# google-research/multinerf

Measured on NVIDIA H100. Metric: train-step rays/sec @16384 rays x (64+64+32) samples, higher is better.
Workload: dtype bf16

## Files before the change

### multinerf_b200/csrc/chain.cu

```cuda
#include <stdlib.h>
#include <string.h>

#include <algorithm>

#include "tc_common.cuh"

namespace mnrf {

constexpr int CH_W = 256;
constexpr int CH_ROWS = 128;
constexpr int CH_KBLK = CH_ROWS * 128;
constexpr int CH_WBLK = CH_W * 128;
constexpr int CH_SLOT = CH_WBLK + CH_KBLK;
constexpr int CH_SLOTS = 3;
constexpr int CH_ACT = 4 * CH_KBLK;
constexpr int CH_THREADS = 384;
constexpr int CH_MAX_LAYERS = MNRF_CHAIN_MAX_LAYERS;
constexpr int CH_SMEM = CH_ACT + CH_SLOTS * CH_SLOT + CH_MAX_LAYERS * CH_W * 4  + 256  +
                        1024 ;
static_assert(CH_SMEM <= 232448, "shared memory budget");

struct alignas(64) ChainMaps {
  CUtensorMap stream;
  CUtensorMap w[CH_MAX_LAYERS];
  CUtensorMap out[CH_MAX_LAYERS];
};

struct ChainLayer {
  int n_stream, stream_col0, stream_kb0;
  int n_res, res_kb0;
  int store;
  const float* bias;
  uint32_t* maskbits;
  int64_t ldmaskbits;
  float* colsum;
};

struct ChainParams {
  int num_layers;
  int64_t m;
  int64_t num_units;
  ChainLayer layer[CH_MAX_LAYERS];
  const float* head_w;
  const float* head_b;
  float* head_out;
};

__device__ __forceinline__ uint32_t pack_bf16_relu(float lo, float hi) {
  uint32_t r;
  asm("cvt.rn.relu.bf16x2.f32 %0, %1, %2;" : "=r"(r) : "f"(hi), "f"(lo));
  return r;
}

template <int MODE, int NH>
__global__ void __launch_bounds__(CH_THREADS, 1)
mlp_chain_kernel(const __grid_constant__ ChainMaps maps, const ChainParams p) {
  extern __shared__ uint8_t smem_dyn[];
  uint8_t* smem = reinterpret_cast<uint8_t*>((reinterpret_cast<uintptr_t>(smem_dyn) + 1023) & ~uintptr_t(1023));
  uint8_t* act = smem;
  uint8_t* ring = smem + CH_ACT;
  float* cs_s = reinterpret_cast<float*>(ring + CH_SLOTS * CH_SLOT);
  uint64_t* full_bar = reinterpret_cast<uint64_t*>(cs_s + CH_MAX_LAYERS * CH_W);
  uint64_t* empty_bar = full_bar + CH_SLOTS;

  const int warp = threadIdx.x >> 5;
  const int lane = threadIdx.x & 31;
  const int wg = threadIdx.x >> 7;

  if (threadIdx.x == 0) {
    bool any_stream = false;
    for (int j = 0; j < p.num_layers; ++j) {
      prefetch_tmap(&maps.w[j]);
      if (p.layer[j].store) prefetch_tmap(&maps.out[j]);
      any_stream |= p.layer[j].n_stream > 0;
    }
    if (any_stream) prefetch_tmap(&maps.stream);
    for (int i = 0; i < CH_SLOTS; ++i) { mbar_init(&full_bar[i], 1); mbar_init(&empty_bar[i], 8); }
    fence_barrier_init();
  }
  if (MODE == 1)
    for (int i = threadIdx.x; i < CH_MAX_LAYERS * CH_W; i += CH_THREADS) cs_s[i] = 0.f;
  __syncthreads();
  pdl_launch_dependents();
  pdl_wait();

  if (wg == 0) {
    setmaxnreg_dec<40>();
    if (threadIdx.x == 0) {
      uint32_t slot = 0, phase = 0;
      for (int64_t unit = blockIdx.x; unit < p.num_units; unit += gridDim.x) {
        const int row0 = (int)(unit * CH_ROWS);
        for (int j = 0; j < p.num_layers; ++j) {
          const ChainLayer& L = p.layer[j];
          for (int s = 0; s < L.n_res + L.n_stream; ++s) {
            const bool streamed = s >= L.n_res;
            const int si = s - L.n_res;
            mbar_wait(&empty_bar[slot], phase ^ 1, 1);
            mbar_expect_tx(&full_bar[slot], streamed ? CH_SLOT : CH_WBLK);
            uint8_t* sl = ring + slot * CH_SLOT;
            const int kb = streamed ? L.stream_kb0 + si : L.res_kb0 + s;
            tma_load_2d(sl, &maps.w[j], &full_bar[slot], kb * 64, 0);
            if (streamed) tma_load_2d(sl + CH_WBLK, &maps.stream, &full_bar[slot], L.stream_col0 + si * 64, row0);
            if (++slot == CH_SLOTS) { slot = 0; phase ^= 1; }
          }
        }
      }
    }
  } else {
    setmaxnreg_inc<232>();
    const int c = wg - 1;
    const int w = warp & 3;
    const int r_in = 64 * c + 16 * w + (lane >> 2);
    const int cq = 2 * (lane & 3);
    const uint32_t ring_s = smem_u32(ring), act_s = smem_u32(act);
    const bool lead = (threadIdx.x & 127) == 0;
    uint32_t slot = 0, phase = 0;
    float acc[CH_W / 2];
    for (int64_t unit = blockIdx.x; unit < p.num_units; unit += gridDim.x) {
      for (int j = 0; j < p.num_layers; ++j) {
        const ChainLayer& L = p.layer[j];
        const bool last = (j == p.num_layers - 1);
        const bool do_head = (MODE == 0) && last && p.head_w != nullptr;
        int prev = -1;
        fence_acc(acc);
        for (int s = 0; s < L.n_res + L.n_stream; ++s) {
          const bool streamed = s >= L.n_res;
          mbar_wait(&full_bar[slot], phase, 3);
          const uint32_t sl = ring_s + slot * CH_SLOT;
          const uint32_t a0 = (streamed ? sl + CH_WBLK : act_s + s * CH_KBLK) + c * (64 * 128);
          wgmma_fence();
#pragma unroll
          for (int k = 0; k < 64 / WGMMA_K; ++k)
            Wgmma<CH_W, 0, 0>::mma(acc, make_smem_desc(a0 + k * (WGMMA_K * 2), 0, 1024),
                                   make_smem_desc(sl + k * (WGMMA_K * 2), 0, 1024), (s > 0 || k > 0) ? 1u : 0u);
          wgmma_commit();
          wgmma_wait<1>();
          if (prev >= 0 && lane == 0) mbar_arrive(&empty_bar[prev]);
          prev = (int)slot;
          if (++slot == CH_SLOTS) { slot = 0; phase ^= 1; }
        }
        wgmma_wait<0>();
        fence_acc(acc);
        if (prev >= 0 && lane == 0) mbar_arrive(&empty_bar[prev]);

        if (lead) tma_store_wait_read<0>();
        named_bar_sync(1 + c, 128);
        int64_t rows[2];
        bool row_ok[2];
#pragma unroll
        for (int h = 0; h < 2; ++h) {
          rows[h] = unit * CH_ROWS + r_in + 8 * h;
          row_ok[h] = rows[h] < p.m;
        }
        uint32_t bits[2] = {0u, 0u};
        float hdot[NH][2];
#pragma unroll
        for (int o = 0; o < NH; ++o) hdot[o][0] = hdot[o][1] = 0.f;
#pragma unroll
        for (int i = 0; i < CH_W / 8; ++i) {
          const int col = 8 * i + cq;
          float v[2][2];
#pragma unroll
          for (int h = 0; h < 2; ++h) { v[h][0] = acc[4 * i + 2 * h]; v[h][1] = acc[4 * i + 2 * h + 1]; }
          uint32_t o[2];
          if (MODE == 0) {
            const float2 b = __ldg(reinterpret_cast<const float2*>(L.bias + col));
#pragma unroll
            for (int h = 0; h < 2; ++h) {
              v[h][0] += b.x;
              v[h][1] += b.y;
              bits[h] |= ((v[h][0] > 0.f ? 1u : 0u) | (v[h][1] > 0.f ? 2u : 0u)) << (col & 31);
              o[h] = pack_bf16_relu(v[h][0], v[h][1]);
            }
            if (do_head) {
#pragma unroll
              for (int oo = 0; oo < NH; ++oo) {
                const float2 hw = __ldg(reinterpret_cast<const float2*>(p.head_w + oo * CH_W + col));
#pragma unroll
                for (int h = 0; h < 2; ++h) hdot[oo][h] += bf16_lo(o[h]) * hw.x + bf16_hi(o[h]) * hw.y;
              }
            }
          } else {
#pragma unroll
            for (int h = 0; h < 2; ++h) {
              if (L.maskbits) {
                const uint32_t wd = row_ok[h] ? __ldg(L.maskbits + rows[h] * L.ldmaskbits + (col >> 5)) : 0u;
                if (!((wd >> (col & 31)) & 1u)) v[h][0] = 0.f;
                if (!((wd >> ((col + 1) & 31)) & 1u)) v[h][1] = 0.f;
              }
              o[h] = pack_bf16(v[h][0], v[h][1]);
            }
            if (L.colsum) {
              float s0 = v[0][0] + v[1][0], s1 = v[0][1] + v[1][1];
#pragma unroll
              for (int sh = 4; sh < 32; sh <<= 1) {
                s0 += __shfl_xor_sync(0xffffffffu, s0, sh);
                s1 += __shfl_xor_sync(0xffffffffu, s1, sh);
              }
              if (lane < 4) { atomicAdd(cs_s + j * CH_W + col, s0); atomicAdd(cs_s + j * CH_W + col + 1, s1); }
            }
          }
#pragma unroll
          for (int h = 0; h < 2; ++h) {
            const int r = r_in + 8 * h;
            st_shared_u32(act_s + (col >> 6) * CH_KBLK + r * 128 + ((((col & 63) >> 3) ^ (r & 7)) << 4) + (cq << 1), o[h]);
// ... 131 lines not shown
```

### multinerf_b200/csrc/gemm_tc.cu

```cuda
#include <cuda.h>

#include <stdlib.h>
#include <string.h>

#include <algorithm>

#include "tc_common.cuh"

namespace mnrf {

constexpr int BLOCK_M = 128;
constexpr int BLOCK_K = 64;
constexpr int A_STAGE_BYTES = BLOCK_M * BLOCK_K * 2;
constexpr int NUM_THREADS = 384;
constexpr int CS_MAX = 1024;
constexpr int gemm_stages(int bn) { return bn == 256 ? 4 : bn == 128 ? 6 : 8; }
constexpr int STAGING_BLOCK_BYTES = 64 * 128;
constexpr int staging_blocks(int mode, int bn, bool ts) {
  return !ts ? 0 : (mode == MNRF_GEMM_FWD && bn >= 128) ? 2 : 1;
}
constexpr int mask_words(int bn) { return bn >= 128 ? bn / 32 : 0; }
constexpr int MASK_BUFS = 2;
constexpr int dgrad_smem_bytes(int bn) { return 8 * bn * 4 + MASK_BUFS * BLOCK_M * mask_words(bn) * 4; }
constexpr int SIDE_SCRATCH = 96 * 8;
constexpr int smem_bytes(int mode, int bn, bool ts, bool side) {
  return gemm_stages(bn) * (A_STAGE_BYTES + bn * BLOCK_K * 2) + 2 * staging_blocks(mode, bn, ts) * STAGING_BLOCK_BYTES +
         (mode == MNRF_GEMM_DGRAD ? dgrad_smem_bytes(bn) : 0) + (side ? SIDE_SCRATCH * 4 : 0) + 256  +
         1024 ;
}

struct GemmParams {
  int mode, act;
  int64_t m;
  int n, k;
  int num_m_blocks, num_n_blocks, num_splits, kblocks_per_split, num_k_blocks;
  int64_t ldc, ldmask;
  const float* bias;
  const float* rowv;
  const float* colv;
  const __nv_bfloat16* mask;
  uint32_t* maskbits;
  int64_t ldmaskbits;
  int64_t mask_mod;
  int mask_tma;
  const __nv_bfloat16* addend;
  int64_t ldadd;
  float* colsum;
  float* bsum;
  const float* side_w;
  float* side_aw;
  void* out;
};

template <int STAGES, int STAGE_BYTES, int CHUNKS, int NT, bool WEIGHTED>
__device__ __forceinline__ void wgrad_side_sums(const GemmParams& p, int t, uint32_t ring, uint64_t* full_bar,
                                                uint64_t* empty_bar, uint32_t scratch) {
  constexpr int G = NT / CHUNKS;
  constexpr int COLS = CHUNKS * 8;
  static_assert(NT % CHUNKS == 0 && NT % 32 == 0, "side-sum warps tile the chunks");
  const int lane = t & 31;
  const int c = t % CHUNKS, g0 = t / CHUNKS;
  ring += (c >> 3) * (BLOCK_K * 128) + ((c & 7) << 4);
  const int total_tiles = p.num_m_blocks * p.num_n_blocks * p.num_splits;
  const int every = WEIGHTED ? p.num_n_blocks : p.num_m_blocks;
  const int step = every * G;
  uint32_t slot = 0;
  for (int tile = blockIdx.x; tile < total_tiles; tile += gridDim.x) {
    const int n_blk = tile % p.num_n_blocks;
    const int rest = tile / p.num_n_blocks;
    const int m_blk = rest % p.num_m_blocks;
    const int split = rest / p.num_m_blocks;
    const int kb0 = split * p.kblocks_per_split;
    const int kb1 = min(p.num_k_blocks, kb0 + p.kblocks_per_split);
    const int own = WEIGHTED ? n_blk : m_blk;
    float acc[8];
#pragma unroll
    for (int e = 0; e < 8; ++e) acc[e] = 0.f;
    for (int kb = kb0; kb < kb1; ++kb, ++slot) {
      float wlo = 0.f, whi = 0.f;
      if (WEIGHTED) {
        const int r0 = kb * BLOCK_K + lane;
        if (r0 < p.k) wlo = __ldg(p.side_w + r0);
        if (r0 + 32 < p.k) whi = __ldg(p.side_w + r0 + 32);
      }
      mbar_wait(&full_bar[slot % STAGES], (slot / STAGES) & 1, 6);
      const uint32_t base = ring + (slot % STAGES) * STAGE_BYTES;
#pragma unroll(WEIGHTED ? 2 : 1)
      for (int r0 = own; r0 < BLOCK_K; r0 += step) {
        const int r = r0 + every * g0;
        float w = 1.f;
        if (WEIGHTED) {
          const float wl = __shfl_sync(0xffffffffu, wlo, r & 31), wh = __shfl_sync(0xffffffffu, whi, r & 31);
          w = r < 32 ? wl : wh;
        }
        if (r < BLOCK_K) {
          const uint4 v = ld_shared_v4((base + r * 128) ^ ((r & 7) << 4));
          const uint32_t u[4] = {v.x, v.y, v.z, v.w};
#pragma unroll
          for (int q = 0; q < 4; ++q) {
            acc[2 * q] = fmaf(w, bf16_lo(u[q]), acc[2 * q]);
            acc[2 * q + 1] = fmaf(w, bf16_hi(u[q]), acc[2 * q + 1]);
          }
        }
      }
      __syncwarp();
      if (lane == 0) mbar_arrive(&empty_bar[slot % STAGES]);
    }
    if (own < BLOCK_K && kb0 < kb1) {
      if (NT > 32) named_bar_sync(4, NT); else __syncwarp();
#pragma unroll
      for (int e = 0; e < 8; ++e) st_shared_u32(scratch + (t * 8 + e) * 4, __float_as_uint(acc[e]));
      if (NT > 32) named_bar_sync(4, NT); else __syncwarp();
      const int64_t col0 = WEIGHTED ? (int64_t)m_blk * BLOCK_M : (int64_t)n_blk * COLS;
      float* out = WEIGHTED ? p.side_aw : p.bsum;
      for (int col = t; col < COLS; col += NT) {
        if (WEIGHTED && col0 + col >= p.m) break;
        float sum = 0.f;
#pragma unroll
        for (int g = 0; g < G; ++g) sum += __uint_as_float(ld_shared_u32(scratch + (g * COLS + col) * 4));
        atomicAdd(out + col0 + col, sum);
      }
    }
  }
}

template <int MODE, int BN, bool TS, bool SIDE, bool SMOOTH = false>
__global__ void __launch_bounds__(NUM_THREADS, 1)
gemm_tc_kernel(const __grid_constant__ CUtensorMap tmap_a, const __grid_constant__ CUtensorMap tmap_b,
               const __grid_constant__ CUtensorMap tmap_c, const __grid_constant__ CUtensorMap tmap_m,
               const GemmParams p) {
  constexpr int STAGES = gemm_stages(BN);
  constexpr int B_STAGE = BN * BLOCK_K * 2;
  constexpr bool kWgrad = (MODE == MNRF_GEMM_WGRAD);
  constexpr bool kDgrad = (MODE == MNRF_GEMM_DGRAD);
  constexpr int NACC = BN / 2;
  constexpr int SB = staging_blocks(MODE, BN, TS);
  constexpr int MW = mask_words(BN);
  static_assert(SB < 2 || (BN / 64) % 2 == 0, "block j of every tile must use staging block j % SB");
  static_assert(!SIDE || kWgrad, "side sums are a WGRAD feature");
  static_assert(!SMOOTH || (TS && !kWgrad), "smooth activations are FWD / DGRAD epilogues of the staged store");
  extern __shared__ uint8_t smem_dyn[];
  uint8_t* smem = reinterpret_cast<uint8_t*>((reinterpret_cast<uintptr_t>(smem_dyn) + 1023) & ~uintptr_t(1023));
  uint8_t* smem_a = smem;
  uint8_t* smem_b = smem + STAGES * A_STAGE_BYTES;
  uint8_t* smem_c = smem_b + STAGES * B_STAGE;
  float* cs_s = reinterpret_cast<float*>(smem_c + 2 * SB * STAGING_BLOCK_BYTES);
  float* side_s = cs_s;
  uint32_t* mask_s = reinterpret_cast<uint32_t*>(cs_s + (kDgrad ? 8 * BN : SIDE ? SIDE_SCRATCH : 0));
  uint64_t* full_bar = reinterpret_cast<uint64_t*>(mask_s + (kDgrad ? MASK_BUFS * BLOCK_M * MW : 0));
  uint64_t* empty_bar = full_bar + STAGES;
  uint64_t* mask_full = empty_bar + STAGES;
  uint64_t* mask_empty = mask_full + MASK_BUFS;

  const int warp = threadIdx.x >> 5;
  const int lane = threadIdx.x & 31;
  const int wg = threadIdx.x >> 7;
  const int total_tiles = p.num_m_blocks * p.num_n_blocks * p.num_splits;
  const bool do_cs = kDgrad && p.colsum != nullptr;
  const bool mask_tma = kDgrad && p.mask_tma;

  if (threadIdx.x == 0) {
    prefetch_tmap(&tmap_a);
    prefetch_tmap(&tmap_b);
    if (TS) prefetch_tmap(&tmap_c);
    if (mask_tma) prefetch_tmap(&tmap_m);
    for (int i = 0; i < STAGES; ++i) {
      mbar_init(&full_bar[i], 1);
      mbar_init(&empty_bar[i], 8 + (!SIDE ? 0 : !p.side_aw ? 3 : p.bsum ? 3 : 2));
    }
    for (int i = 0; i < MASK_BUFS; ++i) {
      mbar_init(&mask_full[i], 1);
      mbar_init(&mask_empty[i], 8);
    }
    fence_barrier_init();
  }
  if (do_cs)
    for (int i = threadIdx.x; i < 8 * BN; i += NUM_THREADS) cs_s[i] = 0.f;
  __syncthreads();
  pdl_launch_dependents();
  pdl_wait();

  if (wg == 0) {
    setmaxnreg_dec<40>();
    if (threadIdx.x == 0) {
      const uint32_t stage_bytes = A_STAGE_BYTES + B_STAGE;
      uint32_t stage = 0, phase = 0;
      for (int tile = blockIdx.x, it = 0; tile < total_tiles; tile += gridDim.x, ++it) {
        const int n_blk = tile % p.num_n_blocks;
        const int rest = tile / p.num_n_blocks;
        const int m_blk = rest % p.num_m_blocks;
        const int split = rest / p.num_m_blocks;
        const int kb0 = split * p.kblocks_per_split;
        const int kb1 = min(p.num_k_blocks, kb0 + p.kblocks_per_split);
        if (mask_tma) {
          const int mb = it % MASK_BUFS;
          mbar_wait(&mask_empty[mb], ((it / MASK_BUFS) & 1) ^ 1, 4);
          mbar_expect_tx(&mask_full[mb], BLOCK_M * MW * 4);
          const int64_t r0 = (int64_t)m_blk * BLOCK_M;
          tma_load_2d(mask_s + mb * (BLOCK_M * MW), &tmap_m, &mask_full[mb], n_blk * (BN / 32),
                      (int)(p.mask_mod > 0 ? r0 % p.mask_mod : r0));
        }
        for (int kb = kb0; kb < kb1; ++kb) {
          mbar_wait(&empty_bar[stage], phase ^ 1, 1);
          mbar_expect_tx(&full_bar[stage], stage_bytes);
          uint8_t* sa = smem_a + stage * A_STAGE_BYTES;
          uint8_t* sb = smem_b + stage * B_STAGE;
          if (!kWgrad) {
            tma_load_2d(sa, &tmap_a, &full_bar[stage], kb * BLOCK_K, m_blk * BLOCK_M);
            tma_load_2d(sb, &tmap_b, &full_bar[stage], kb * BLOCK_K, n_blk * BN);
          } else {
#pragma unroll
            for (int a = 0; a < BLOCK_M / 64; ++a)
              tma_load_2d(sa + a * (BLOCK_K * 128), &tmap_a, &full_bar[stage], m_blk * BLOCK_M + a * 64, kb * BLOCK_K);
#pragma unroll
            for (int a = 0; a < BN / 64; ++a)
              tma_load_2d(sb + a * (BLOCK_K * 128), &tmap_b, &full_bar[stage], n_blk * BN + a * 64, kb * BLOCK_K);
          }
          if (++stage == STAGES) { stage = 0; phase ^= 1; }
        }
      }
    } else if (SIDE && warp > 0) {
      const uint32_t scratch = smem_u32(side_s);
      if (!p.side_aw) {
        wgrad_side_sums<STAGES, B_STAGE, BN / 8, 96, false>(p, threadIdx.x - 32, smem_u32(smem_b), full_bar, empty_bar,
                                                            scratch);
      } else if (warp >= 2) {
        wgrad_side_sums<STAGES, A_STAGE_BYTES, BLOCK_M / 8, 64, true>(p, threadIdx.x - 64, smem_u32(smem_a), full_bar,
                                                                      empty_bar, scratch + 32 * 8 * 4);
      } else if (p.bsum) {
        wgrad_side_sums<STAGES, B_STAGE, BN / 8, 32, false>(p, lane, smem_u32(smem_b), full_bar, empty_bar, scratch);
      }
    }
  } else {
    setmaxnreg_inc<232>();
    const int c = wg - 1;
    const int w = warp & 3;
    const int r_in = 64 * c + 16 * w + (lane >> 2);
    const int cq = 2 * (lane & 3);
    uint32_t stage = 0, phase = 0;
    float acc[NACC];
    const uint32_t cs_lane = smem_u32(cs_s) + ((warp - 4) * BN + cq + ((lane >> 2) & 1)) * 4;
    for (int tile = blockIdx.x, it = 0; tile < total_tiles; tile += gridDim.x, ++it) {
      const int n_blk = tile % p.num_n_blocks;
      const int rest = tile / p.num_n_blocks;
      const int m_blk = rest % p.num_m_blocks;
      const int split = rest / p.num_m_blocks;
      const int kb0 = split * p.kblocks_per_split;
      const int kb1 = min(p.num_k_blocks, kb0 + p.kblocks_per_split);
      int prev = -1;
      fence_acc(acc);
      for (int kb = kb0; kb < kb1; ++kb) {
        mbar_wait(&full_bar[stage], phase, 3);
        const uint32_t sa = smem_u32(smem_a + stage * A_STAGE_BYTES);
        const uint32_t sb = smem_u32(smem_b + stage * B_STAGE);
        wgmma_fence();
#pragma unroll
        for (int k = 0; k < BLOCK_K / WGMMA_K; ++k) {
          uint64_t adesc, bdesc;
          if (!kWgrad) {
            adesc = make_smem_desc(sa + c * (64 * 128) + k * (WGMMA_K * 2), 0, 1024);
            bdesc = make_smem_desc(sb + k * (WGMMA_K * 2), 0, 1024);
          } else {
            adesc = make_smem_desc(sa + c * (BLOCK_K * 128) + k * (WGMMA_K * 128), BLOCK_K * 128, 1024);
            bdesc = make_smem_desc(sb + k * (WGMMA_K * 128), BLOCK_K * 128, 1024);
          }
          Wgmma<BN, kWgrad ? 1 : 0, kWgrad ? 1 : 0>::mma(acc, adesc, bdesc, (kb > kb0 || k > 0) ? 1u : 0u);
        }
        wgmma_commit();
        wgmma_wait<1>();
        if (prev >= 0 && lane == 0) mbar_arrive(&empty_bar[prev]);
        prev = (int)stage;
        if (++stage == STAGES) { stage = 0; phase ^= 1; }
      }
      wgmma_wait<0>();
      fence_acc(acc);
      if (prev >= 0 && lane == 0) mbar_arrive(&empty_bar[prev]);

      const int ncol0 = n_blk * BN;
      if (MODE == MNRF_GEMM_WGRAD) {
#pragma unroll
        for (int h = 0; h < 2; ++h) {
          const int64_t row = (int64_t)m_blk * BLOCK_M + r_in + 8 * h;
          if (row >= p.m) continue;
          float* dst = reinterpret_cast<float*>(p.out) + row * p.ldc + ncol0 + cq;
#pragma unroll
          for (int i = 0; i < BN / 8; ++i) atomicAdd(reinterpret_cast<float2*>(dst + 8 * i), make_float2(acc[4 * i + 2 * h], acc[4 * i + 2 * h + 1]));
        }
        continue;
      }
      const bool leader = (threadIdx.x & 127) == 0;
      const uint32_t c_row = smem_u32(smem_c) + c * (SB * STAGING_BLOCK_BYTES) + (r_in - 64 * c) * 128 + (cq << 1);
      int64_t rows[2];
      bool row_ok[2];
      float rv[2] = {0.f, 0.f};
      const uint32_t* mrow[2] = {nullptr, nullptr};
#pragma unroll
      for (int h = 0; h < 2; ++h) {
        rows[h] = (int64_t)m_blk * BLOCK_M + r_in + 8 * h;
        row_ok[h] = rows[h] < p.m;
        if (MODE == MNRF_GEMM_DGRAD && row_ok[h]) {
          if (p.rowv) rv[h] = p.rowv[rows[h]];
          if (p.maskbits && !mask_tma)
            mrow[h] = p.maskbits + (p.mask_mod > 0 ? rows[h] % p.mask_mod : rows[h]) * p.ldmaskbits;
        }
      }
      const uint32_t m_row = smem_u32(mask_s) + ((it % MASK_BUFS) * BLOCK_M + r_in) * (MW * 4);
      if (mask_tma) mbar_wait(&mask_full[it % MASK_BUFS], (it / MASK_BUFS) & 1, 5);
      uint32_t bits[2] = {0u, 0u};
      uint32_t mw[2] = {0u, 0u};
#pragma unroll
      for (int i = 0; i < BN / 8; ++i) {
        const int col = ncol0 + 8 * i + cq;
        if (TS && SB == 1 && (i & 7) == 0) {
          if (leader) tma_store_wait_read<0>();
          named_bar_sync(2 + c, 128);
        }
        if (MODE == MNRF_GEMM_DGRAD && p.maskbits && (i & 3) == 0) {
#pragma unroll
          for (int h = 0; h < 2; ++h)
            mw[h] = mask_tma ? ld_shared_u32(m_row + (8 * h * MW + (i >> 2)) * 4)
                             : row_ok[h] ? __ldg(mrow[h] + (col >> 5)) : 0u;
        }
        float v[2][2];
#pragma unroll
        for (int h = 0; h < 2; ++h) { v[h][0] = acc[4 * i + 2 * h]; v[h][1] = acc[4 * i + 2 * h + 1]; }
        if (MODE == MNRF_GEMM_FWD) {
          if (p.bias) {
            const float2 b = __ldg(reinterpret_cast<const float2*>(p.bias + col));
#pragma unroll
            for (int h = 0; h < 2; ++h) { v[h][0] += b.x; v[h][1] += b.y; }
          }
          if constexpr (SMOOTH) {
#pragma unroll
            for (int h = 0; h < 2; ++h) {
              if (p.mask && row_ok[h])
                *reinterpret_cast<uint32_t*>(const_cast<__nv_bfloat16*>(p.mask) + rows[h] * p.ldmask + col) =
                    pack_bf16(v[h][0], v[h][1]);
              v[h][0] = act_fwd(p.act, v[h][0]);
              v[h][1] = act_fwd(p.act, v[h][1]);
            }
          } else if (p.act == MNRF_ACT_RELU) {
#pragma unroll
            for (int h = 0; h < 2; ++h)
#pragma unroll
              for (int e = 0; e < 2; ++e) {
                v[h][e] = fmaxf(v[h][e], 0.f);
                bits[h] |= (v[h][e] > 0.f ? 1u : 0u) << ((8 * i + cq + e) & 31);
              }
          }
        } else {
          float2 cv = make_float2(0.f, 0.f);
          if (p.rowv) cv = __ldg(reinterpret_cast<const float2*>(p.colv + col));
#pragma unroll
          for (int h = 0; h < 2; ++h) {
            if (p.rowv) { v[h][0] += rv[h] * cv.x; v[h][1] += rv[h] * cv.y; }
            if constexpr (SMOOTH) {
              if (row_ok[h]) {
                const int64_t zr = p.mask_mod > 0 ? rows[h] % p.mask_mod : rows[h];
                const uint32_t zz = __ldg(reinterpret_cast<const unsigned int*>(p.mask + zr * p.ldmask + col));
                v[h][0] *= act_d1(p.act, bf16_lo(zz));
                v[h][1] *= act_d1(p.act, bf16_hi(zz));
              }
            } else if (p.maskbits) {
              if (!((mw[h] >> (col & 31)) & 1u)) v[h][0] = 0.f;
              if (!((mw[h] >> ((col + 1) & 31)) & 1u)) v[h][1] = 0.f;
            } else if (p.mask && row_ok[h]) {
              const uint32_t mm = __ldg(reinterpret_cast<const unsigned int*>(p.mask + rows[h] * p.ldmask + col));
              if (!(bf16_lo(mm) > 0.f)) v[h][0] = 0.f;
              if (!(bf16_hi(mm) > 0.f)) v[h][1] = 0.f;
            }
            if (p.addend && row_ok[h]) {
              const uint32_t aa = __ldg(reinterpret_cast<const unsigned int*>(p.addend + rows[h] * p.ldadd + col));
              v[h][0] += bf16_lo(aa);
              v[h][1] += bf16_hi(aa);
            }
          }
          if (do_cs) {
            const bool hi = (lane >> 2) & 1;
            const float s0 = v[0][0] + v[1][0], s1 = v[0][1] + v[1][1];
            float t = (hi ? s1 : s0) + __shfl_xor_sync(0xffffffffu, hi ? s0 : s1, 4);
            t += __shfl_xor_sync(0xffffffffu, t, 8);
            t += __shfl_xor_sync(0xffffffffu, t, 16);
            if (lane < 8) {
              const uint32_t a = cs_lane + 8 * i * 4;
              st_shared_u32(a, __float_as_uint(__uint_as_float(ld_shared_u32(a)) + t));
            }
          }
        }
#pragma unroll
        for (int h = 0; h < 2; ++h) {
          if (TS) {
            st_shared_u32(c_row + ((i >> 3) & (SB - 1)) * STAGING_BLOCK_BYTES + h * (8 * 128) +
                              (((i & 7) ^ ((lane >> 2) & 7)) << 4),
                          pack_bf16(v[h][0], v[h][1]));
          } else if (row_ok[h]) {
            *reinterpret_cast<uint32_t*>(reinterpret_cast<__nv_bfloat16*>(p.out) + rows[h] * p.ldc + col) =
                pack_bf16(v[h][0], v[h][1]);
          }
        }
        if (MODE == MNRF_GEMM_FWD && p.act == MNRF_ACT_RELU && p.maskbits && (i & 3) == 3) {
#pragma unroll
          for (int h = 0; h < 2; ++h) {
            bits[h] |= __shfl_xor_sync(0xffffffffu, bits[h], 1);
            bits[h] |= __shfl_xor_sync(0xffffffffu, bits[h], 2);
            if ((lane & 3) == ((i >> 2) & 3) && row_ok[h]) p.maskbits[rows[h] * p.ldmaskbits + (col >> 5)] = bits[h];
            bits[h] = 0u;
          }
        }
        if (TS && (i & 7) == 7) {
          fence_proxy_async();
          if (SB == 2 && leader) tma_store_wait_read<0>();
          named_bar_sync(2 + c, 128);
          if (leader) {
            tma_store_2d(&tmap_c, smem_c + (c * SB + ((i >> 3) & (SB - 1))) * STAGING_BLOCK_BYTES, ncol0 + 8 * (i & ~7),
                         (int)((int64_t)m_blk * BLOCK_M + 64 * c));
            tma_store_commit();
          }
        }
      }
      if (mask_tma) {
        __syncwarp();
        if (lane == 0) mbar_arrive(&mask_empty[it % MASK_BUFS]);
      }
      const int next = tile + (int)gridDim.x;
      if (do_cs && (next >= total_tiles || next % p.num_n_blocks != n_blk)) {
        named_bar_sync(1, 2 * 128);
        for (int j = threadIdx.x - 128; j < BN; j += 2 * 128) {
          float s = 0.f;
#pragma unroll
          for (int sw = 0; sw < 8; ++sw) {
            s += cs_s[sw * BN + j];
            cs_s[sw * BN + j] = 0.f;
          }
          atomicAdd(p.colsum + ncol0 + j, s);
        }
        named_bar_sync(1, 2 * 128);
      }
    }
    if (TS && (threadIdx.x & 127) == 0) tma_store_wait_all();
  }
}

template <int MODE, int BN, bool TS, bool SIDE, bool SMOOTH>
static int launch_gemm_tc(int grid, const CUtensorMap& ta, const CUtensorMap& tb, const CUtensorMap& tc,
                          const CUtensorMap& tm, const GemmParams& p, cudaStream_t stream) {
  static bool attr_set = false;
  constexpr int kSmem = smem_bytes(MODE, BN, TS, SIDE);
  static_assert(kSmem <= 232448, "shared memory budget");
  auto kern = gemm_tc_kernel<MODE, BN, TS, SIDE, SMOOTH>;
  if (!attr_set) {
    MNRF_CUDA(cudaFuncSetAttribute(kern, cudaFuncAttributeMaxDynamicSharedMemorySize, kSmem));
    attr_set = true;
  }
  cudaLaunchConfig_t cfg = {};
  cfg.gridDim = dim3(grid); cfg.blockDim = dim3(NUM_THREADS);
  cfg.dynamicSmemBytes = kSmem; cfg.stream = stream;
  cudaLaunchAttribute attr[1];
  attr[0].id = cudaLaunchAttributeProgrammaticStreamSerialization;
  attr[0].val.programmaticStreamSerializationAllowed = 1;
  cfg.attrs = attr; cfg.numAttrs = pdl_enabled() ? 1 : 0;
  MNRF_CUDA(cudaLaunchKernelEx(&cfg, kern, ta, tb, tc, tm, p));
  return 0;
}

int gemm_tc_smooth_launch(int mode, int block_n, int grid, const CUtensorMap& ta, const CUtensorMap& tb,
                          const CUtensorMap& tc, const GemmParams& p, cudaStream_t stream);

#ifndef MNRF_GEMM_TC_SMOOTH_UNIT
static int pick_block_n(int n) {
  const int cands[] = {256, 128, 64, 32, 16};
  for (int c : cands)
    if (n % c == 0) return c;
  return 0;
}

int gemm_tc_launch(const mnrf_gemm_desc* d, const mnrf_bf16* a, const mnrf_bf16* b, const float* bias,
                   const float* rowv, const float* colv, const mnrf_bf16* mask, uint32_t* maskbits,
                   float* colsum, const mnrf_bf16* addend, void* out, cudaStream_t stream, float* bsum,
                   const float* side_w, float* side_aw, mnrf_bf16* z, int64_t ldz) {
  MNRF_CHECK(d->mode == MNRF_GEMM_WGRAD || d->k % BLOCK_K == 0,
             "mnrf_gemm(tc): reduction length %d must be a multiple of %d", d->k, BLOCK_K);
  MNRF_CHECK(d->lda % 8 == 0 && d->ldb % 8 == 0 && ((uintptr_t)a % 16) == 0 && ((uintptr_t)b % 16) == 0,
             "mnrf_gemm(tc): operands must be 16-byte aligned with ld %% 8 == 0");
  GemmParams p{};
  p.mode = d->mode; p.act = d->act; p.m = d->m; p.n = d->n; p.k = d->k;
  const int block_n = pick_block_n(d->n);
  MNRF_CHECK(block_n > 0, "mnrf_gemm(tc): N=%d must be a multiple of 16", d->n);
  if (d->mode == MNRF_GEMM_WGRAD)
    MNRF_CHECK(block_n >= 64, "mnrf_gemm(tc): WGRAD needs N %% 64 == 0 (MN-major 128-byte atoms), N=%d", d->n);
  p.num_m_blocks = (int)((d->m + BLOCK_M - 1) / BLOCK_M);
  p.num_n_blocks = d->n / block_n;
  p.num_k_blocks = (d->k + BLOCK_K - 1) / BLOCK_K;
  p.ldc = d->ldc; p.ldmask = d->ldmask;
  p.bias = bias; p.rowv = rowv; p.colv = colv;
  p.mask = reinterpret_cast<const __nv_bfloat16*>(mask);
  p.out = out;
  p.maskbits = maskbits;
  p.ldmaskbits = d->ldmaskbits;
  p.mask_mod = d->mask_mod;
  p.addend = reinterpret_cast<const __nv_bfloat16*>(addend);
  p.ldadd = d->ldadd;
  if (addend) MNRF_CHECK(d->mode == MNRF_GEMM_DGRAD && d->ldadd % 2 == 0 && ((uintptr_t)addend % 4) == 0,
                         "mnrf_gemm(tc): addend is a DGRAD input with 4-byte aligned rows");
  p.colsum = colsum;
  if (colsum) MNRF_CHECK(d->mode == MNRF_GEMM_DGRAD && d->n <= CS_MAX,
                         "mnrf_gemm(tc): colsum is a DGRAD output of at most %d columns", CS_MAX);
  const bool side = bsum != nullptr || side_aw != nullptr;
  if (side) MNRF_CHECK(d->mode == MNRF_GEMM_WGRAD && (side_w == nullptr) == (side_aw == nullptr),
                       "mnrf_gemm(tc): side sums are WGRAD outputs; side_w and side_aw come together");
  p.bsum = bsum; p.side_w = side_w; p.side_aw = side_aw;
  if (maskbits) {
    MNRF_CHECK(d->mode != MNRF_GEMM_WGRAD, "mnrf_gemm(tc): maskbits make no sense for WGRAD");
    MNRF_CHECK(d->n % 32 == 0 && block_n % 32 == 0 && d->ldmaskbits * 32 >= d->n,
               "mnrf_gemm(tc): maskbits need N %% 32 == 0 and ldmaskbits >= N/32");
  }
  const bool smooth = d->mode != MNRF_GEMM_WGRAD && (d->act == MNRF_ACT_SOFTPLUS || d->act == MNRF_ACT_SILU);
  if (smooth) {
    MNRF_CHECK(!maskbits && !mask, "mnrf_gemm(tc): a smooth activation takes z, not a ReLU mask");
    MNRF_CHECK(d->mode == MNRF_GEMM_FWD || z, "mnrf_gemm(tc): the DGRAD of a smooth activation needs z");
    MNRF_CHECK(!z || (ldz % 2 == 0 && ((uintptr_t)z % 4) == 0), "mnrf_gemm(tc): z must be 4-byte aligned");
  }
  if (smooth) {
    p.mask = reinterpret_cast<const __nv_bfloat16*>(z);
    p.ldmask = ldz;
  }
  if (bias) MNRF_CHECK(((uintptr_t)bias % 8) == 0, "mnrf_gemm(tc): bias must be 8-byte aligned");
  if (colv) MNRF_CHECK(((uintptr_t)colv % 8) == 0, "mnrf_gemm(tc): colv must be 8-byte aligned");
  const int workers = mnrf_num_sms();
  p.num_splits = 1;
  if (d->mode == MNRF_GEMM_WGRAD) {
    const int out_tiles = p.num_m_blocks * p.num_n_blocks;
    const int max_splits = std::min(std::max(1, (2 * workers) / out_tiles), p.num_k_blocks);
    int splits = max_splits;
    for (int sp = 1; sp <= max_splits; ++sp) {
      const int items = out_tiles * sp;
      const int rounds = (items + workers - 1) / workers;
      if (items * 100 >= rounds * workers * 95) { splits = sp; break; }
    }
    p.num_splits = splits;
  }
  p.kblocks_per_split = (p.num_k_blocks + p.num_splits - 1) / p.num_splits;
  p.num_splits = (p.num_k_blocks + p.kblocks_per_split - 1) / p.kblocks_per_split;
  if (d->mode != MNRF_GEMM_WGRAD) {
    MNRF_CHECK(d->ldc % 2 == 0 && ((uintptr_t)out % 4) == 0, "mnrf_gemm(tc): bf16 output must be 4-byte aligned");
    if (mask) MNRF_CHECK(d->ldmask % 2 == 0 && ((uintptr_t)mask % 4) == 0, "mnrf_gemm(tc): mask must be 4-byte aligned");
  } else {
    MNRF_CHECK(d->ldc % 2 == 0 && ((uintptr_t)out % 8) == 0, "mnrf_gemm(tc): fp32 output must be 8-byte aligned");
  }

  const bool ts = d->mode != MNRF_GEMM_WGRAD && block_n >= 64 && ((uintptr_t)out % 16) == 0 && d->ldc % 8 == 0;
  MNRF_CHECK(!smooth || ts, "mnrf_gemm(tc): a smooth activation needs N %% 64 == 0 and a 16-byte aligned output "
             "with a row pitch that is a multiple of 8");
  CUtensorMap ta, tb, tc;
  if (d->mode != MNRF_GEMM_WGRAD) {
    if (make_tmap(&ta, a, d->m, d->k, d->lda, BLOCK_K, BLOCK_M)) return 1;
    if (make_tmap(&tb, b, d->n, d->k, d->ldb, BLOCK_K, block_n)) return 1;
  } else {
    if (make_tmap(&ta, a, d->k, d->m, d->lda, 64, BLOCK_K)) return 1;
    if (make_tmap(&tb, b, d->k, d->n, d->ldb, 64, BLOCK_K)) return 1;
  }
  if (ts) {
    if (make_tmap(&tc, out, d->m, d->n, d->ldc, 64, 64)) return 1;
  } else {
    tc = tb;
  }
  CUtensorMap tm = tb;
  p.mask_tma = d->mode == MNRF_GEMM_DGRAD && maskbits && mask_words(block_n) > 0 && d->ldmaskbits % 4 == 0 &&
               ((uintptr_t)maskbits % 16) == 0 && (d->mask_mod == 0 || d->mask_mod % BLOCK_M == 0);
  if (p.mask_tma &&
      make_tmap(&tm, maskbits, d->mask_mod > 0 ? d->mask_mod : d->m, d->n / 32, d->ldmaskbits,
                mask_words(block_n), BLOCK_M, CU_TENSOR_MAP_DATA_TYPE_UINT32, 4,
                CU_TENSOR_MAP_SWIZZLE_NONE))
    return 1;
  const int total_tiles = p.num_m_blocks * p.num_n_blocks * p.num_splits;
  const int grid = std::min(total_tiles, workers);
  if (grid == 0) return 0;
#define MNRF_LAUNCH_TC3(MODE_, BN_, TS_, SIDE_)                                                       \
  do {                                                                                                \
    if (int rc = launch_gemm_tc<MODE_, BN_, TS_, SIDE_, false>(grid, ta, tb, tc, tm, p, stream)) return rc; \
  } while (0)
#define MNRF_LAUNCH_TC2(MODE_, BN_)                                                                   \
  do {                                                                                                \
    if (side) MNRF_LAUNCH_TC3(MODE_, BN_, false, MODE_ == MNRF_GEMM_WGRAD && BN_ >= 64);              \
    else if (ts) MNRF_LAUNCH_TC3(MODE_, BN_, MODE_ != MNRF_GEMM_WGRAD && BN_ >= 64, false);           \
    else MNRF_LAUNCH_TC3(MODE_, BN_, false, false);                                                   \
  } while (0)
#define MNRF_LAUNCH_TC(MODE_)                                                                         \
  do {                                                                                                \
    switch (block_n) {                                                                                \
      case 256: MNRF_LAUNCH_TC2(MODE_, 256); break;                                                   \
      case 128: MNRF_LAUNCH_TC2(MODE_, 128); break;                                                   \
      case 64: MNRF_LAUNCH_TC2(MODE_, 64); break;                                                     \
      case 32: if (MODE_ != MNRF_GEMM_WGRAD) MNRF_LAUNCH_TC2(MODE_, 32); break;                       \
      default: if (MODE_ != MNRF_GEMM_WGRAD) MNRF_LAUNCH_TC2(MODE_, 16); break;                       \
    }                                                                                                 \
  } while (0)
  if (smooth) {
    if (int rc = gemm_tc_smooth_launch(d->mode, block_n, grid, ta, tb, tc, p, stream)) return rc;
  } else if (d->mode == MNRF_GEMM_FWD) MNRF_LAUNCH_TC(MNRF_GEMM_FWD);
  else if (d->mode == MNRF_GEMM_DGRAD) MNRF_LAUNCH_TC(MNRF_GEMM_DGRAD);
  else MNRF_LAUNCH_TC(MNRF_GEMM_WGRAD);
  MNRF_LAUNCH_CHECK();
  return 0;
}
#endif

}
```

### multinerf_b200/csrc/tc_common.cuh

```cuda
#pragma once

#include <cuda.h>
#include <stdlib.h>

#include "common.cuh"
#include "wgmma.cuh"

namespace mnrf {

constexpr int WGMMA_K = 16;

__device__ __forceinline__ uint32_t smem_u32(const void* p) {
  return static_cast<uint32_t>(__cvta_generic_to_shared(p));
}
__device__ __forceinline__ void mbar_init(uint64_t* bar, uint32_t count) {
  asm volatile("mbarrier.init.shared::cta.b64 [%0], %1;" ::"r"(smem_u32(bar)), "r"(count));
}
__device__ __forceinline__ void mbar_expect_tx(uint64_t* bar, uint32_t bytes) {
  asm volatile("mbarrier.arrive.expect_tx.shared::cta.b64 _, [%0], %1;" ::"r"(smem_u32(bar)), "r"(bytes) : "memory");
}
__device__ __forceinline__ void mbar_arrive(uint64_t* bar) {
  asm volatile("mbarrier.arrive.shared::cta.b64 _, [%0];" ::"r"(smem_u32(bar)) : "memory");
}
__device__ __forceinline__ bool mbar_try_wait(uint64_t* bar, uint32_t parity) {
  uint32_t ok;
  asm volatile(
      "{\n"
      ".reg .pred p;\n"
      "mbarrier.try_wait.parity.shared::cta.b64 p, [%1], %2;\n"
      "selp.u32 %0, 1, 0, p;\n"
      "}\n"
      : "=r"(ok) : "r"(smem_u32(bar)), "r"(parity) : "memory");
  return ok != 0;
}
__device__ __forceinline__ void mbar_wait(uint64_t* bar, uint32_t parity, int tag) {
  (void)tag;
  if (mbar_try_wait(bar, parity)) return;
  const long long t0 = clock64();
  while (!mbar_try_wait(bar, parity)) {
    if (clock64() - t0 > 4000000000LL) __trap();
  }
}
__device__ __forceinline__ void fence_barrier_init() {
  asm volatile("fence.mbarrier_init.release.cluster;" ::: "memory");
}
__device__ __forceinline__ void fence_proxy_async() {
  asm volatile("fence.proxy.async.shared::cta;" ::: "memory");
}
__device__ __forceinline__ void tma_load_2d(void* smem_dst, const CUtensorMap* map, uint64_t* bar,
                                            int c0, int c1) {
  asm volatile(
      "cp.async.bulk.tensor.2d.shared::cluster.global.mbarrier::complete_tx::bytes [%0], [%1, {%3, %4}], [%2];"
      :: "r"(smem_u32(smem_dst)), "l"(reinterpret_cast<uint64_t>(map)), "r"(smem_u32(bar)), "r"(c0), "r"(c1)
      : "memory");
}
__device__ __forceinline__ void tma_prefetch_2d(const CUtensorMap* map, int c0, int c1) {
  asm volatile("cp.async.bulk.prefetch.tensor.2d.L2.global.tile [%0, {%1, %2}];"
               :: "l"(reinterpret_cast<uint64_t>(map)), "r"(c0), "r"(c1) : "memory");
}
__device__ __forceinline__ void tma_store_2d(const CUtensorMap* map, const void* smem_src, int c0, int c1) {
  asm volatile("cp.async.bulk.tensor.2d.global.shared::cta.bulk_group [%0, {%2, %3}], [%1];"
               :: "l"(reinterpret_cast<uint64_t>(map)), "r"(smem_u32(smem_src)), "r"(c0), "r"(c1) : "memory");
}
__device__ __forceinline__ void tma_store_commit() { asm volatile("cp.async.bulk.commit_group;" ::: "memory"); }
template <int N>
__device__ __forceinline__ void tma_store_wait_read() {
  asm volatile("cp.async.bulk.wait_group.read %0;" ::"n"(N) : "memory");
}
__device__ __forceinline__ void tma_store_wait_all() { asm volatile("cp.async.bulk.wait_group 0;" ::: "memory"); }
__device__ __forceinline__ void prefetch_tmap(const CUtensorMap* map) {
  asm volatile("prefetch.tensormap [%0];" ::"l"(reinterpret_cast<uint64_t>(map)) : "memory");
}
__device__ __forceinline__ void st_shared_u32(uint32_t addr, uint32_t v) {
  asm volatile("st.shared.b32 [%0], %1;" ::"r"(addr), "r"(v) : "memory");
}
__device__ __forceinline__ uint32_t ld_shared_u32(uint32_t addr) {
  uint32_t v;
  asm volatile("ld.shared.b32 %0, [%1];" : "=r"(v) : "r"(addr) : "memory");
  return v;
}
__device__ __forceinline__ uint4 ld_shared_v4(uint32_t addr) {
  uint4 v;
  asm volatile("ld.shared.v4.b32 {%0, %1, %2, %3}, [%4];"
               : "=r"(v.x), "=r"(v.y), "=r"(v.z), "=r"(v.w) : "r"(addr) : "memory");
  return v;
}
__device__ __forceinline__ void named_bar_sync(int id, int count) {
  asm volatile("bar.sync %0, %1;" ::"r"(id), "r"(count) : "memory");
}

template <int R>
__device__ __forceinline__ void setmaxnreg_dec() { asm volatile("setmaxnreg.dec.sync.aligned.u32 %0;" ::"n"(R)); }
template <int R>
__device__ __forceinline__ void setmaxnreg_inc() { asm volatile("setmaxnreg.inc.sync.aligned.u32 %0;" ::"n"(R)); }

__device__ __forceinline__ void wgmma_fence() { asm volatile("wgmma.fence.sync.aligned;" ::: "memory"); }
__device__ __forceinline__ void wgmma_commit() { asm volatile("wgmma.commit_group.sync.aligned;" ::: "memory"); }
template <int N>
__device__ __forceinline__ void wgmma_wait() { asm volatile("wgmma.wait_group.sync.aligned %0;" ::"n"(N) : "memory"); }
template <int R>
__device__ __forceinline__ void fence_acc(float (&d)[R]) {
#pragma unroll
  for (int i = 0; i < R; ++i) asm volatile("" : "+f"(d[i])::"memory");
}
__device__ __forceinline__ void pdl_wait() { asm volatile("griddepcontrol.wait;" ::: "memory"); }
__device__ __forceinline__ void pdl_launch_dependents() { asm volatile("griddepcontrol.launch_dependents;" ::: "memory"); }

__device__ __forceinline__ uint64_t make_smem_desc(uint32_t saddr, uint32_t lbo_bytes, uint32_t sbo_bytes) {
  uint64_t d = 0;
  d |= (uint64_t)((saddr >> 4) & 0x3fff);
  d |= (uint64_t)((lbo_bytes >> 4) & 0x3fff) << 16;
  d |= (uint64_t)((sbo_bytes >> 4) & 0x3fff) << 32;
  d |= (uint64_t)1 << 62;
  return d;
}

typedef CUresult (*EncodeTiledFn)(CUtensorMap*, CUtensorMapDataType, cuuint32_t, void*, const cuuint64_t*,
                                  const cuuint64_t*, const cuuint32_t*, const cuuint32_t*,
                                  CUtensorMapInterleave, CUtensorMapSwizzle, CUtensorMapL2promotion,
                                  CUtensorMapFloatOOBfill);

inline bool pdl_enabled() {
  static const bool on = getenv("MNRF_PDL") != nullptr && atoi(getenv("MNRF_PDL")) != 0;
  return on;
}

inline EncodeTiledFn get_encode_fn() {
  static EncodeTiledFn fn = nullptr;
  if (fn) return fn;
  void* ptr = nullptr;
  cudaDriverEntryPointQueryResult qres;
  if (cudaGetDriverEntryPoint("cuTensorMapEncodeTiled", &ptr, cudaEnableDefault, &qres) != cudaSuccess ||
      qres != cudaDriverEntryPointSuccess)
    return nullptr;
  fn = reinterpret_cast<EncodeTiledFn>(ptr);
  return fn;
}

inline int make_tmap(CUtensorMap* map, const void* base, int64_t rows, int64_t cols, int64_t ld,
                     int box_cols, int box_rows,
                     CUtensorMapDataType dtype = CU_TENSOR_MAP_DATA_TYPE_BFLOAT16, int elem_bytes = 2,
                     CUtensorMapSwizzle swizzle = CU_TENSOR_MAP_SWIZZLE_128B) {
  EncodeTiledFn fn = get_encode_fn();
  MNRF_CHECK(fn, "cuTensorMapEncodeTiled is not available from the driver");
  cuuint64_t dims[2] = {(cuuint64_t)cols, (cuuint64_t)rows};
  cuuint64_t strides[1] = {(cuuint64_t)ld * elem_bytes};
  cuuint32_t box[2] = {(cuuint32_t)box_cols, (cuuint32_t)box_rows};
  cuuint32_t estr[2] = {1, 1};
  CUresult r = fn(map, dtype, 2, const_cast<void*>(base), dims, strides, box, estr,
                  CU_TENSOR_MAP_INTERLEAVE_NONE, swizzle, CU_TENSOR_MAP_L2_PROMOTION_L2_256B,
                  CU_TENSOR_MAP_FLOAT_OOB_FILL_NONE);
  MNRF_CHECK(r == CUDA_SUCCESS, "cuTensorMapEncodeTiled failed (%d): rows=%lld cols=%lld ld=%lld box=%dx%d base=%p",
             (int)r, (long long)rows, (long long)cols, (long long)ld, box_cols, box_rows, base);
  return 0;
}


}
```

Measured before the change: 243,600.

## Offload staged TMA store and relu mask bits to producer-warpgroup side warps

The staged-store epilogue now writes the bf16 output tile into the just-consumed A/B ring stage buffers plus a smaller private area, instead of dedicated staging buffers. Idle producer-warpgroup warps issue the TMA stores, compute the forward relu mask bits from shared memory, and release the ring stage. Consumers no longer wait on TMA reads per 64-column block. The relu is fused into the bf16 conversion instruction. The aim is to shrink shared memory, cut consumer-side sync and shuffle work in the epilogue, and overlap stores with the next tile. In exchange the last ring stage stays held until the stores drain, and new staged/released barriers add cross-warpgroup coupling.

```diff
diff --git a/multinerf_b200/csrc/chain.cu b/multinerf_b200/csrc/chain.cu
--- a/multinerf_b200/csrc/chain.cu
+++ b/multinerf_b200/csrc/chain.cu
@@ -45,12 +45,6 @@
   const float* head_b;
   float* head_out;
 };
-
-__device__ __forceinline__ uint32_t pack_bf16_relu(float lo, float hi) {
-  uint32_t r;
-  asm("cvt.rn.relu.bf16x2.f32 %0, %1, %2;" : "=r"(r) : "f"(hi), "f"(lo));
-  return r;
-}
 
 template <int MODE, int NH>
 __global__ void __launch_bounds__(CH_THREADS, 1)
diff --git a/multinerf_b200/csrc/gemm_tc.cu b/multinerf_b200/csrc/gemm_tc.cu
--- a/multinerf_b200/csrc/gemm_tc.cu
+++ b/multinerf_b200/csrc/gemm_tc.cu
@@ -16,15 +16,20 @@
 constexpr int CS_MAX = 1024;
 constexpr int gemm_stages(int bn) { return bn == 256 ? 4 : bn == 128 ? 6 : 8; }
 constexpr int STAGING_BLOCK_BYTES = 64 * 128;
-constexpr int staging_blocks(int mode, int bn, bool ts) {
-  return !ts ? 0 : (mode == MNRF_GEMM_FWD && bn >= 128) ? 2 : 1;
+constexpr int own_blocks(int bn, bool ts) { return ts ? bn / 64 - 1 - bn / 128 : 0; }
+template <int BN>
+__device__ __forceinline__ uint32_t staged_block(uint32_t a_stage, uint32_t b_stage, uint32_t own, int c, int j) {
+  constexpr int OWN = own_blocks(BN, true);
+  return j == 0     ? a_stage + c * STAGING_BLOCK_BYTES
+         : j <= OWN ? own + c * STAGING_BLOCK_BYTES
+                    : b_stage + (c * (BN / 128) + j - 1 - OWN) * STAGING_BLOCK_BYTES;
 }
 constexpr int mask_words(int bn) { return bn >= 128 ? bn / 32 : 0; }
 constexpr int MASK_BUFS = 2;
 constexpr int dgrad_smem_bytes(int bn) { return 8 * bn * 4 + MASK_BUFS * BLOCK_M * mask_words(bn) * 4; }
 constexpr int SIDE_SCRATCH = 96 * 8;
 constexpr int smem_bytes(int mode, int bn, bool ts, bool side) {
-  return gemm_stages(bn) * (A_STAGE_BYTES + bn * BLOCK_K * 2) + 2 * staging_blocks(mode, bn, ts) * STAGING_BLOCK_BYTES +
+  return gemm_stages(bn) * (A_STAGE_BYTES + bn * BLOCK_K * 2) + 2 * own_blocks(bn, ts) * STAGING_BLOCK_BYTES +
          (mode == MNRF_GEMM_DGRAD ? dgrad_smem_bytes(bn) : 0) + (side ? SIDE_SCRATCH * 4 : 0) + 256  +
          1024 ;
 }
@@ -124,6 +129,63 @@
   }
 }
 
+template <int MODE, int BN, int STAGES>
+__device__ __forceinline__ void staged_tile_side(const GemmParams& p, int t, const CUtensorMap* tmap_c,
+                                                 uint32_t ring_a, uint32_t ring_b, uint32_t own, uint64_t* empty_bar,
+                                                 uint64_t* staged_bar, uint64_t* released_bar) {
+  constexpr int MWT = BN / 32;
+  constexpr int UNITS = BLOCK_M * MWT;
+  const bool fwd_bits = MODE == MNRF_GEMM_FWD && p.act == MNRF_ACT_RELU && p.maskbits;
+  const int total_tiles = p.num_m_blocks * p.num_n_blocks;
+  uint32_t slot = 0;
+  for (int tile = blockIdx.x, it = 0; tile < total_tiles; tile += gridDim.x, ++it) {
+    const int n_blk = tile % p.num_n_blocks;
+    const int m_blk = tile / p.num_n_blocks;
+    slot += p.num_k_blocks;
+    const int held = (slot - 1) % STAGES;
+    const uint32_t a_st = ring_a + held * A_STAGE_BYTES, b_st = ring_b + held * (BN * BLOCK_K * 2);
+    const int64_t row0 = (int64_t)m_blk * BLOCK_M;
+    auto unit_row = [&](int r, int w) {
+      return staged_block<BN>(a_st, b_st, own, r >> 6, w >> 1) + (r & 63) * 128;
+    };
+    mbar_wait(staged_bar, it & 1, 7);
+    if (t == 0) {
+#pragma unroll
+      for (int c = 0; c < 2; ++c)
+#pragma unroll
+        for (int j = 0; j < BN / 64; ++j)
+          tma_store_2d(tmap_c, staged_block<BN>(a_st, b_st, own, c, j), n_blk * BN + 64 * j, (int)(row0 + 64 * c));
+      tma_store_commit();
+    }
+    if (fwd_bits) {
+      for (int u = t; u < UNITS; u += 96) {
+        const int r = u / MWT, w = u % MWT;
+        if (row0 + r >= p.m) break;
+        const uint32_t base = unit_row(r, w);
+        uint4 v[4];
+#pragma unroll
+        for (int q = 0; q < 4; ++q) v[q] = ld_shared_v4(base + (((4 * (w & 1) + q) ^ (r & 7)) << 4));
+        uint32_t word = 0u;
+#pragma unroll
+        for (int q = 0; q < 4; ++q) {
+          const uint32_t x[4] = {v[q].x, v[q].y, v[q].z, v[q].w};
+#pragma unroll
+          for (int e = 0; e < 4; ++e)
+            word |= ((bf16_lo(x[e]) > 0.f ? 1u : 0u) | (bf16_hi(x[e]) > 0.f ? 2u : 0u)) << (8 * q + 2 * e);
+        }
+        p.maskbits[(row0 + r) * p.ldmaskbits + n_blk * MWT + w] = word;
+      }
+      named_bar_sync(4, 96);
+    }
+    if (t == 0) {
+      tma_store_wait_read<0>();
+      mbar_arrive_cnt(&empty_bar[held], 8);
+      mbar_arrive(released_bar);
+    }
+  }
+  if (t == 0) tma_store_wait_all();
+}
+
 template <int MODE, int BN, bool TS, bool SIDE, bool SMOOTH = false>
 __global__ void __launch_bounds__(NUM_THREADS, 1)
 gemm_tc_kernel(const __grid_constant__ CUtensorMap tmap_a, const __grid_constant__ CUtensorMap tmap_b,
@@ -134,23 +196,25 @@
   constexpr bool kWgrad = (MODE == MNRF_GEMM_WGRAD);
   constexpr bool kDgrad = (MODE == MNRF_GEMM_DGRAD);
   constexpr int NACC = BN / 2;
-  constexpr int SB = staging_blocks(MODE, BN, TS);
+  constexpr int OWN = own_blocks(BN, TS);
   constexpr int MW = mask_words(BN);
-  static_assert(SB < 2 || (BN / 64) % 2 == 0, "block j of every tile must use staging block j % SB");
   static_assert(!SIDE || kWgrad, "side sums are a WGRAD feature");
-  static_assert(!SMOOTH || (TS && !kWgrad), "smooth activations are FWD / DGRAD epilogues of the staged store");
+  static_assert(!TS || (!kWgrad && BN >= 64), "the staged store takes whole 64-column blocks of a bf16 output");
+  static_assert(!SMOOTH || TS, "smooth activations are FWD / DGRAD epilogues of the staged store");
   extern __shared__ uint8_t smem_dyn[];
   uint8_t* smem = reinterpret_cast<uint8_t*>((reinterpret_cast<uintptr_t>(smem_dyn) + 1023) & ~uintptr_t(1023));
   uint8_t* smem_a = smem;
   uint8_t* smem_b = smem + STAGES * A_STAGE_BYTES;
-  uint8_t* smem_c = smem_b + STAGES * B_STAGE;
-  float* cs_s = reinterpret_cast<float*>(smem_c + 2 * SB * STAGING_BLOCK_BYTES);
+  uint8_t* smem_own = smem_b + STAGES * B_STAGE;
+  float* cs_s = reinterpret_cast<float*>(smem_own + 2 * OWN * STAGING_BLOCK_BYTES);
   float* side_s = cs_s;
   uint32_t* mask_s = reinterpret_cast<uint32_t*>(cs_s + (kDgrad ? 8 * BN : SIDE ? SIDE_SCRATCH : 0));
   uint64_t* full_bar = reinterpret_cast<uint64_t*>(mask_s + (kDgrad ? MASK_BUFS * BLOCK_M * MW : 0));
   uint64_t* empty_bar = full_bar + STAGES;
   uint64_t* mask_full = empty_bar + STAGES;
   uint64_t* mask_empty = mask_full + MASK_BUFS;
+  uint64_t* staged_bar = mask_empty + MASK_BUFS;
+  uint64_t* released_bar = staged_bar + 1;
 
   const int warp = threadIdx.x >> 5;
   const int lane = threadIdx.x & 31;
@@ -172,6 +236,8 @@
       mbar_init(&mask_full[i], 1);
       mbar_init(&mask_empty[i], 8);
     }
+    mbar_init(staged_bar, 8);
+    mbar_init(released_bar, 1);
     fence_barrier_init();
   }
   if (do_cs)
@@ -230,6 +296,10 @@
       } else if (p.bsum) {
         wgrad_side_sums<STAGES, B_STAGE, BN / 8, 32, false>(p, lane, smem_u32(smem_b), full_bar, empty_bar, scratch);
       }
+    } else if (warp > 0) {
+      if constexpr (TS)
+        staged_tile_side<MODE, BN, STAGES>(p, threadIdx.x - 32, &tmap_c, smem_u32(smem_a), smem_u32(smem_b),
+                                           smem_u32(smem_own), empty_bar, staged_bar, released_bar);
     }
   } else {
     setmaxnreg_inc<232>();
@@ -274,7 +344,7 @@
       }
       wgmma_wait<0>();
       fence_acc(acc);
-      if (prev >= 0 && lane == 0) mbar_arrive(&empty_bar[prev]);
+      if (!TS && prev >= 0 && lane == 0) mbar_arrive(&empty_bar[prev]);
 
       const int ncol0 = n_blk * BN;
       if (MODE == MNRF_GEMM_WGRAD) {
@@ -288,8 +358,9 @@
         }
         continue;
       }
-      const bool leader = (threadIdx.x & 127) == 0;
-      const uint32_t c_row = smem_u32(smem_c) + c * (SB * STAGING_BLOCK_BYTES) + (r_in - 64 * c) * 128 + (cq << 1);
+      const uint32_t a_st = smem_u32(smem_a + prev * A_STAGE_BYTES), b_st = smem_u32(smem_b + prev * B_STAGE);
+      const uint32_t t_row = (r_in - 64 * c) * 128 + (cq << 1);
+      if (TS && it > 0) mbar_wait(released_bar, (it - 1) & 1, 8);
       int64_t rows[2];
       bool row_ok[2];
       float rv[2] = {0.f, 0.f};
@@ -311,10 +382,7 @@
 #pragma unroll
       for (int i = 0; i < BN / 8; ++i) {
         const int col = ncol0 + 8 * i + cq;
-        if (TS && SB == 1 && (i & 7) == 0) {
-          if (leader) tma_store_wait_read<0>();
-          named_bar_sync(2 + c, 128);
-        }
+        if (TS && i == 8 * (1 + OWN)) named_bar_sync(1, 2 * 128);
         if (MODE == MNRF_GEMM_DGRAD && p.maskbits && (i & 3) == 0) {
 #pragma unroll
           for (int h = 0; h < 2; ++h)
@@ -324,6 +392,7 @@
         float v[2][2];
 #pragma unroll
         for (int h = 0; h < 2; ++h) { v[h][0] = acc[4 * i + 2 * h]; v[h][1] = acc[4 * i + 2 * h + 1]; }
+        bool relu_cvt = false;
         if (MODE == MNRF_GEMM_FWD) {
           if (p.bias) {
             const float2 b = __ldg(reinterpret_cast<const float2*>(p.bias + col));
@@ -339,6 +408,8 @@
               v[h][0] = act_fwd(p.act, v[h][0]);
               v[h][1] = act_fwd(p.act, v[h][1]);
             }
+          } else if (TS && p.act == MNRF_ACT_RELU) {
+            relu_cvt = true;
           } else if (p.act == MNRF_ACT_RELU) {
 #pragma unroll
             for (int h = 0; h < 2; ++h)
@@ -389,16 +460,16 @@
         }
 #pragma unroll
         for (int h = 0; h < 2; ++h) {
+          const uint32_t o = relu_cvt ? pack_bf16_relu(v[h][0], v[h][1]) : pack_bf16(v[h][0], v[h][1]);
           if (TS) {
-            st_shared_u32(c_row + ((i >> 3) & (SB - 1)) * STAGING_BLOCK_BYTES + h * (8 * 128) +
+            st_shared_u32(staged_block<BN>(a_st, b_st, smem_u32(smem_own), c, i >> 3) + t_row + h * (8 * 128) +
                               (((i & 7) ^ ((lane >> 2) & 7)) << 4),
-                          pack_bf16(v[h][0], v[h][1]));
+                          o);
           } else if (row_ok[h]) {
-            *reinterpret_cast<uint32_t*>(reinterpret_cast<__nv_bfloat16*>(p.out) + rows[h] * p.ldc + col) =
-                pack_bf16(v[h][0], v[h][1]);
-          }
-        }
-        if (MODE == MNRF_GEMM_FWD && p.act == MNRF_ACT_RELU && p.maskbits && (i & 3) == 3) {
+            *reinterpret_cast<uint32_t*>(reinterpret_cast<__nv_bfloat16*>(p.out) + rows[h] * p.ldc + col) = o;
+          }
+        }
+        if (!TS && MODE == MNRF_GEMM_FWD && p.act == MNRF_ACT_RELU && p.maskbits && (i & 3) == 3) {
 #pragma unroll
           for (int h = 0; h < 2; ++h) {
             bits[h] |= __shfl_xor_sync(0xffffffffu, bits[h], 1);
@@ -407,16 +478,11 @@
             bits[h] = 0u;
           }
         }
-        if (TS && (i & 7) == 7) {
-          fence_proxy_async();
-          if (SB == 2 && leader) tma_store_wait_read<0>();
-          named_bar_sync(2 + c, 128);
-          if (leader) {
-            tma_store_2d(&tmap_c, smem_c + (c * SB + ((i >> 3) & (SB - 1))) * STAGING_BLOCK_BYTES, ncol0 + 8 * (i & ~7),
-                         (int)((int64_t)m_blk * BLOCK_M + 64 * c));
-            tma_store_commit();
-          }
-        }
+      }
+      if (TS) {
+        fence_proxy_async();
+        __syncwarp();
+        if (lane == 0) mbar_arrive(staged_bar);
       }
       if (mask_tma) {
         __syncwarp();
@@ -437,7 +503,6 @@
         named_bar_sync(1, 2 * 128);
       }
     }
-    if (TS && (threadIdx.x & 127) == 0) tma_store_wait_all();
   }
 }
 
@@ -478,8 +543,8 @@
                    const float* rowv, const float* colv, const mnrf_bf16* mask, uint32_t* maskbits,
                    float* colsum, const mnrf_bf16* addend, void* out, cudaStream_t stream, float* bsum,
                    const float* side_w, float* side_aw, mnrf_bf16* z, int64_t ldz) {
-  MNRF_CHECK(d->mode == MNRF_GEMM_WGRAD || d->k % BLOCK_K == 0,
-             "mnrf_gemm(tc): reduction length %d must be a multiple of %d", d->k, BLOCK_K);
+  MNRF_CHECK(d->mode == MNRF_GEMM_WGRAD || (d->k > 0 && d->k % BLOCK_K == 0),
+             "mnrf_gemm(tc): reduction length %d must be a positive multiple of %d", d->k, BLOCK_K);
   MNRF_CHECK(d->lda % 8 == 0 && d->ldb % 8 == 0 && ((uintptr_t)a % 16) == 0 && ((uintptr_t)b % 16) == 0,
              "mnrf_gemm(tc): operands must be 16-byte aligned with ld %% 8 == 0");
   GemmParams p{};
diff --git a/multinerf_b200/csrc/tc_common.cuh b/multinerf_b200/csrc/tc_common.cuh
--- a/multinerf_b200/csrc/tc_common.cuh
+++ b/multinerf_b200/csrc/tc_common.cuh
@@ -21,6 +21,9 @@
 }
 __device__ __forceinline__ void mbar_arrive(uint64_t* bar) {
   asm volatile("mbarrier.arrive.shared::cta.b64 _, [%0];" ::"r"(smem_u32(bar)) : "memory");
+}
+__device__ __forceinline__ void mbar_arrive_cnt(uint64_t* bar, uint32_t count) {
+  asm volatile("mbarrier.arrive.shared::cta.b64 _, [%0], %1;" ::"r"(smem_u32(bar)), "r"(count) : "memory");
 }
 __device__ __forceinline__ bool mbar_try_wait(uint64_t* bar, uint32_t parity) {
   uint32_t ok;
@@ -58,9 +61,12 @@
   asm volatile("cp.async.bulk.prefetch.tensor.2d.L2.global.tile [%0, {%1, %2}];"
                :: "l"(reinterpret_cast<uint64_t>(map)), "r"(c0), "r"(c1) : "memory");
 }
+__device__ __forceinline__ void tma_store_2d(const CUtensorMap* map, uint32_t smem_src, int c0, int c1) {
+  asm volatile("cp.async.bulk.tensor.2d.global.shared::cta.bulk_group [%0, {%2, %3}], [%1];"
+               :: "l"(reinterpret_cast<uint64_t>(map)), "r"(smem_src), "r"(c0), "r"(c1) : "memory");
+}
 __device__ __forceinline__ void tma_store_2d(const CUtensorMap* map, const void* smem_src, int c0, int c1) {
-  asm volatile("cp.async.bulk.tensor.2d.global.shared::cta.bulk_group [%0, {%2, %3}], [%1];"
-               :: "l"(reinterpret_cast<uint64_t>(map)), "r"(smem_u32(smem_src)), "r"(c0), "r"(c1) : "memory");
+  tma_store_2d(map, smem_u32(smem_src), c0, c1);
 }
 __device__ __forceinline__ void tma_store_commit() { asm volatile("cp.async.bulk.commit_group;" ::: "memory"); }
 template <int N>
@@ -87,6 +93,11 @@
 }
 __device__ __forceinline__ void named_bar_sync(int id, int count) {
   asm volatile("bar.sync %0, %1;" ::"r"(id), "r"(count) : "memory");
+}
+__device__ __forceinline__ uint32_t pack_bf16_relu(float lo, float hi) {
+  uint32_t r;
+  asm("cvt.rn.relu.bf16x2.f32 %0, %1, %2;" : "=r"(r) : "f"(hi), "f"(lo));
+  return r;
 }
 
 template <int R>
```

Result: faster. 250,200 (median of 6 runs) (+2.7%).
